# FelipeMartins96/rsoccer-isaac-cleanrl

Hardware: AMD Instinct MI355X
Metric: env-steps/s (num_envs×horizon) at 65 536 envs; PPO wall-clock to 1e8 steps (higher is better)
Workload: dtype f32; 1 GPU; vss_step FULL contract: 65536 fields/GPU, one launch per control step, random actions (BASELINE configs[1]/[2] shape); fields_per_gpu=65536, mode=full, agent_rows_per_field=1, launch=eager ctypes launches, parallelism=fields sharded over 1 GPU(s), no data-path collective

## Files before the change

### rsoccer-isaac-cleanrl_amd/csrc/vss_step.hip

```cpp
#include <hip/hip_runtime.h>
#include <type_traits>
#include <stdint.h>

#include "../../include/vss.h"

#pragma clang fp contract(off)

#if defined(__HIP_DEVICE_COMPILE__) && !defined(__gfx950__)
#error "vss_step.hip targets gfx950 (CDNA4) only: wait_loads() and v_permlane32_swap are gfx950 encodings"
#endif

namespace vss {

constexpr int kWave = 64;
constexpr int kFpw = 32;
constexpr int kRec = 59;

constexpr int NSUB = 2;
#define K_H 0.025f
#define K_HH 0.0125f
#define K_FIELD_HX 0.75f
#define K_FIELD_HY 0.65f
#define K_GOAL_HY 0.2f
#define K_GOAL_BACK_X 0.85f
// ... 312 lines not shown
      ox[k] = up ? b.x[k + 3] : b.x[k];
      oy[k] = up ? b.y[k + 3] : b.y[k];
      ovx[k] = up ? b.vx[k + 3] : b.vx[k];
      ovy[k] = up ? b.vy[k + 3] : b.vy[k];
      contact_walls(ox[k], oy[k], ovx[k], ovy[k], K_ROBOT_R);
      exch(ox[k], b.x[k], b.x[k + 3]);
      exch(oy[k], b.y[k], b.y[k + 3]);
      exch(ovx[k], b.vx[k], b.vx[k + 3]);
      exch(ovy[k], b.vy[k], b.vy[k + 3]);
    }
    contact_walls(b.bx, b.by, b.bvx, b.bvy, K_BALL_R);
  }
#pragma unroll
  for (int k = 0; k < 3; ++k) {
    exch(ow[k], b.w[k], b.w[k + 3]);
    exch(oqz[k], b.qz[k], b.qz[k + 3]);
    exch(oqw[k], b.qw[k], b.qw[k + 3]);
  }
}

__device__ __forceinline__ void wait_loads() { __builtin_amdgcn_s_waitcnt(0x0F70); }

template <class T>
__device__ __forceinline__ T& at(T* base, uint32_t byte_off) {
  using B = typename std::conditional<std::is_const<T>::value, const char, char>::type;
  return *reinterpret_cast<T*>(reinterpret_cast<B*>(base) + byte_off);
}

__device__ __forceinline__ void load_bodies(const float* __restrict__ st, int64_t n, int64_t f0, int fl, Bodies& b) {
  float v[VSS_STATE_CHANNELS];
  const float* q = st + f0 + fl;
#pragma unroll
  for (int c = 0; c < VSS_STATE_CHANNELS; ++c) {
    if (c < VSS_CH_RQX || c >= VSS_CH_RQZ)
      v[c] = *q;
    q += n;
  }
  b.bx = v[VSS_CH_BALL_X]; b.by = v[VSS_CH_BALL_Y]; b.bvx = v[VSS_CH_BALL_VX]; b.bvy = v[VSS_CH_BALL_VY];
#pragma unroll
  for (int i = 0; i < 6; ++i) {
    b.x[i] = v[VSS_CH_RX + i]; b.y[i] = v[VSS_CH_RY + i]; b.qz[i] = v[VSS_CH_RQZ + i]; b.qw[i] = v[VSS_CH_RQW + i];
    b.vx[i] = v[VSS_CH_RVX + i]; b.vy[i] = v[VSS_CH_RVY + i]; b.w[i] = v[VSS_CH_RW + i];
  }
}

__device__ __forceinline__ void store_bodies(float* __restrict__ st, int64_t n, int64_t f0, int fl, const Bodies& b) {
  float v[VSS_STATE_CHANNELS];
  v[VSS_CH_BALL_X] = b.bx; v[VSS_CH_BALL_Y] = b.by; v[VSS_CH_BALL_VX] = b.bvx; v[VSS_CH_BALL_VY] = b.bvy;
#pragma unroll
  for (int i = 0; i < 6; ++i) {
    v[VSS_CH_RX + i] = b.x[i]; v[VSS_CH_RY + i] = b.y[i]; v[VSS_CH_RQZ + i] = b.qz[i]; v[VSS_CH_RQW + i] = b.qw[i];
    v[VSS_CH_RVX + i] = b.vx[i]; v[VSS_CH_RVY + i] = b.vy[i]; v[VSS_CH_RW + i] = b.w[i];
  }
  float* q = st + f0 + fl;
#pragma unroll
  for (int c = 0; c < VSS_STATE_CHANNELS; ++c) {
    if (c < VSS_CH_RQX || c >= VSS_CH_RQZ) *q = v[c];
    q += n;
  }
}

template <int W>
__device__ __forceinline__ void coop_load(const float* __restrict__ g, int nv, float* lds, int lane) {
  const int total = nv * W;
  if constexpr (W % 4 == 0) {
    const float4* g4 = reinterpret_cast<const float4*>(g);
    for (int q = lane; q < total / 4; q += kWave) {
      float4 v = at(g4, 16u * (uint32_t)q);
      int e = q * 4, fl = e / W, k = e - fl * W;
      float* d = lds + fl * kRec + k;
      d[0] = v.x; d[1] = v.y; d[2] = v.z; d[3] = v.w;
    }
  } else {
    const float2* g2 = reinterpret_cast<const float2*>(g);
    for (int q = lane; q < total / 2; q += kWave) {
      float2 v = at(g2, 8u * (uint32_t)q);
      int e = q * 2, fl = e / W, k = e - fl * W;
      float* d = lds + fl * kRec + k;
      d[0] = v.x; d[1] = v.y;
    }
  }
}

template <int W>
__device__ __forceinline__ void coop_store(float* __restrict__ g, int nv, const float* lds, int lane) {
  const int total = nv * W;
  if constexpr (W % 4 == 0) {
    float4* g4 = reinterpret_cast<float4*>(g);
    for (int q = lane; q < total / 4; q += kWave) {
      int e = q * 4, fl = e / W, k = e - fl * W;
      const float* s = lds + fl * kRec + k;
      at(g4, 16u * (uint32_t)q) = make_float4(s[0], s[1], s[2], s[3]);
    }
  } else {
    float2* g2 = reinterpret_cast<float2*>(g);
    for (int q = lane; q < total / 2; q += kWave) {
      int e = q * 2, fl = e / W, k = e - fl * W;
      const float* s = lds + fl * kRec + k;
      at(g2, 8u * (uint32_t)q) = make_float2(s[0], s[1]);
    }
  }
}

template <int A>
__device__ __forceinline__ void write_obs_record(float* rec, const Bodies& b, const float dof[12]) {
  rec[0] = b.bx; rec[1] = b.by; rec[2] = b.bvx; rec[3] = b.bvy;
#pragma unroll
  for (int r = 0; r < 6; ++r) {
    float* o = rec + 4 + 9 * r;
    o[0] = b.x[r]; o[1] = b.y[r]; o[2] = b.vx[r]; o[3] = b.vy[r];
    o[4] = b.qw[r] * b.qw[r] - b.qz[r] * b.qz[r];
    o[5] = 2.0f * b.qw[r] * b.qz[r];
    o[6] = b.w[r]; o[7] = dof[2 * r]; o[8] = dof[2 * r + 1];
  }
  if constexpr (A == 6) {
    float* m = rec + kRec;
#pragma unroll
    for (int k = 0; k < 4; ++k) m[k] = __uint_as_float(__float_as_uint(rec[k]) ^ 0x80000000u);
#pragma unroll
    for (int r = 0; r < 6; ++r)
#pragma unroll
      for (int q = 0; q < 6; ++q)
        m[4 + 6 * r + q] = __uint_as_float(__float_as_uint(rec[4 + 9 * r + q]) ^ 0x80000000u);
  }
}

constexpr int kObsUnroll = 4;
template <int A, int A0 = 0, int REC = obs_rec<A>()>
__device__ __forceinline__ void coop_store_obs(float* __restrict__ out, int nv, const float* lds, const uint32_t* tab,
                                               int lane, bool nt = false) {
  static_assert(A0 + A <= 6 && (A0 == 0 || REC == kRecObs6), "yellow agents read the mirror slots");
  constexpr int Q = 13 * A;
  constexpr int QD = kWave / Q, QR = kWave % Q;
  constexpr uint32_t RB = 4u * REC;
  const int total = nv * Q;
  const uint32_t rb_last = (uint32_t)(nv - 1) * RB;
  int fl = lane / Q, j4 = lane - fl * Q;
  uint32_t rb = (uint32_t)fl * RB;
  const char* L = reinterpret_cast<const char*>(lds);
  float4* o4 = reinterpret_cast<float4*>(out);
  for (int q0 = lane; q0 < total; q0 += kObsUnroll * kWave) {
    float4 v[kObsUnroll];
#pragma unroll
    for (int u = 0; u < kObsUnroll; ++u) {
      const uint2 t = reinterpret_cast<const uint2*>(tab)[13 * A0 + j4];
      const uint32_t r = rb < rb_last ? rb : rb_last;
      v[u].x = *reinterpret_cast<const float*>(L + r + (t.x & 0xffffu));
      v[u].y = *reinterpret_cast<const float*>(L + r + (t.x >> 16));
      v[u].z = *reinterpret_cast<const float*>(L + r + (t.y & 0xffffu));
      v[u].w = *reinterpret_cast<const float*>(L + r + (t.y >> 16));
      j4 += QR;
      rb += QD * RB;
      if (j4 >= Q) { j4 -= Q; rb += RB; }
    }
#pragma unroll
    for (int u = 0; u < kObsUnroll; ++u)
      if (q0 + u * kWave < total) {
        if (nt) {
          typedef float f4v __attribute__((ext_vector_type(4)));
          __builtin_nontemporal_store(f4v{v[u].x, v[u].y, v[u].z, v[u].w},
                                      reinterpret_cast<f4v*>(&at(o4, 16u * (uint32_t)(q0 + u * kWave))));
        } else {
          at(o4, 16u * (uint32_t)(q0 + u * kWave)) = v[u];
        }
      }
  }
}

struct ResetDraws {
  uint32_t k0, k1, field, ctr, ext;
  const float* u;
  uint32_t rounds;
};

template <bool REPLAY>
__device__ __forceinline__ float uval(uint32_t w) { return REPLAY ? __uint_as_float(w) : u01(w); }

template <bool REPLAY>
__device__ __forceinline__ void pos_block(const ResetDraws& d, uint32_t round, uint32_t blk, uint32_t o[4]) {
  if constexpr (REPLAY) {
#pragma unroll
    for (uint32_t i = 0; i < 4; ++i) {
      const uint32_t j = 4u * blk + i;
      o[i] = j < 14u ? __float_as_uint(d.u[14u * round + j]) : 0x3f000000u;
    }
  } else {
    philox(d.k0, d.k1, d.field, d.ctr, ((kPurposePos | d.ext) << 24) | round, blk, o);
  }
}

template <bool REPLAY>
__device__ __forceinline__ void ang_block(const ResetDraws& d, uint32_t rounds_used, uint32_t blk, uint32_t o[4]) {
  if constexpr (REPLAY) {
#pragma unroll
    for (uint32_t i = 0; i < 4; ++i) o[i] = __float_as_uint(d.u[14u * rounds_used + 4u * blk + i]);
  } else {
    philox(d.k0, d.k1, d.field, d.ctr, ((kPurposeAng | d.ext) << 24), blk, o);
  }
}

template <bool REPLAY>
__device__ __forceinline__ void reset_field(Bodies& b, const ResetDraws& d) {
  const float scale_x = 1.5f - 0.14f, scale_y = 1.3f - 0.14f;
  float px[7], py[7];
  uint32_t round = 0;
  for (;; ++round) {
    uint32_t o[16];
#pragma unroll
    for (int blk = 0; blk < 4; ++blk) pos_block<REPLAY>(d, round, (uint32_t)blk, o + 4 * blk);
#pragma unroll
    for (int e = 0; e < 7; ++e) {
      px[e] = (uval<REPLAY>(o[2 * e]) - 0.5f) * scale_x;
      py[e] = (uval<REPLAY>(o[2 * e + 1]) - 0.5f) * scale_y;
    }
    bool close = false;
#pragma unroll
    for (int i = 0; i < 7; ++i)
#pragma unroll
      for (int j = i + 1; j < 7; ++j) {
        float dx = px[i] - px[j], dy = py[i] - py[j];
        close |= dx * dx + dy * dy < __uint_as_float(0x3ba0902du);
      }
    if (!close || round + 1 >= d.rounds) break;
  }
  b.bx = px[0]; b.by = py[0];
  uint32_t o[8];
  ang_block<REPLAY>(d, round + 1, 0u, o);
  ang_block<REPLAY>(d, round + 1, 1u, o + 4);
#pragma unroll
  for (int r = 0; r < 6; ++r) {
    b.x[r] = px[1 + r]; b.y[r] = py[1 + r];
    b.vx[r] = 0.0f; b.vy[r] = 0.0f; b.w[r] = 0.0f;
    float ang = K_TWO_PI * uval<REPLAY>(o[r]) + (-K_PI);
    float sh, ch;
    sincos_small(ang * 0.5f, sh, ch);
    float nrm = sqrtf(sh * sh + ch * ch);
    b.qz[r] = sh / nrm;
    b.qw[r] = ch / nrm;
  }
  b.bvx = uval<REPLAY>(o[6]) - 0.5f;
  b.bvy = uval<REPLAY>(o[7]) - 0.5f;
}

template <bool REPLAY>
__device__ __forceinline__ void reset_field_split(Bodies& b, const ResetDraws& d) {
  const float kMinDist2 = __uint_as_float(0x3ba0902du);
  const bool up = threadIdx.x >= 32;
  const uint32_t blk0 = up ? 2u : 0u;
// ... 128 lines not shown
  const float u1 = u01_open0(w1), u2 = u01(w2);
  const float rad = sqrtf(-2.0f * logf_poly(u1));
  float sz, cz;
  sincos_turn(u2, sz, cz);
  zc = K_OU_SIGMA * (rad * cz);
  zs = K_OU_SIGMA * (rad * sz);
}

template <int MODE>
__device__ __forceinline__ void ou_noise_split(float a[12], uint32_t k0, uint32_t k1, uint32_t field, uint32_t ctr) {
  const bool up = threadIdx.x >= 32;
  float z[12];
  if constexpr (MODE == VSS_MODE_SA) {
    uint32_t p[4], q[4];
    philox(k0, k1, field, ctr, kPurposeOU << 24, up ? 2u : 0u, p);
    philox(k0, k1, field, ctr, kPurposeOU << 24, up ? 2u : 1u, q);
    float c0, s0, c1, s1, c2, s2;
    box_muller(up ? p[0] : p[2], up ? p[1] : p[3], c0, s0);
    box_muller(up ? p[2] : q[0], up ? p[3] : q[1], c1, s1);
    box_muller(q[2], q[3], c2, s2);
    exch(c0, z[2], z[8]);
    exch(s0, z[3], z[9]);
    exch(c1, z[4], z[10]);
    exch(s1, z[5], z[11]);
    float unused;
    exch(c2, z[6], unused);
    exch(s2, z[7], unused);
  } else {
    uint32_t p[4];
    philox(k0, k1, field, ctr, kPurposeOU << 24, up ? 2u : 1u, p);
    float c0, s0, c1, s1;
    box_muller(up ? p[0] : p[2], up ? p[1] : p[3], c0, s0);
    box_muller(p[2], p[3], c1, s1);
    exch(c0, z[6], z[8]);
    exch(s0, z[7], z[9]);
    float unused;
    exch(c1, unused, z[10]);
    exch(s1, unused, z[11]);
  }
  constexpr int NL = MODE == VSS_MODE_SA ? 2 : 6;
#pragma unroll
  for (int k = NL; k < 12; ++k) a[k] = clampf((a[k] - K_OU_THETA * a[k]) + z[k], -1.0f, 1.0f);
}

__device__ __forceinline__ void ou_noise_blue_sa(float a[12], uint32_t k0, uint32_t k1, uint32_t field, uint32_t ctr) {
  const bool up = threadIdx.x >= 32;
  uint32_t w[4];
  philox(k0, k1, field, ctr, kPurposeOU << 24, up ? 1u : 0u, w);
  float zc, zs, z[6];
  box_muller(up ? w[0] : w[2], up ? w[1] : w[3], zc, zs);
  exch(zc, z[2], z[4]);
  exch(zs, z[3], z[5]);
#pragma unroll
  for (int k = 2; k < 6; ++k) a[k] = clampf((a[k] - K_OU_THETA * a[k]) + z[k], -1.0f, 1.0f);
}

template <bool REPLAY>
__device__ __forceinline__ void reset_if_done(bool valid, int64_t done, const ResetDraws& rd, Bodies& b,
                                              const float a[12], float dof[12]) {
#pragma unroll
  for (int k = 0; k < 12; ++k) dof[k] = a[k];
  if (valid && done) {
    reset_field_split<REPLAY>(b, rd);
#pragma unroll
    for (int k = 0; k < 12; ++k) dof[k] = dof[k] * 0.0f;
  }
}

struct BatchIn {
  int64_t progress, reset_prev;
  uint32_t ctr;
  Bodies b;
  float4 blk[3];
  float2 lrn[2];
};

struct StepArgs {
  int64_t n;
  vss_params p;
  vss_state s;
  vss_step_io io;
  vss_replay_draws rd;
  uint32_t rd_rounds;
  uint32_t nt_obs;
};

template <int MODE>
__device__ __forceinline__ void load_batch(const StepArgs& args, int64_t f0, int nv, int fl, int lane, BatchIn& in) {
  constexpr int NL = MODE == VSS_MODE_SA ? 2 : 6;
  in.progress = 0;
  in.reset_prev = 0;
  in.ctr = 0;
  in.b = {};
  if (fl < nv) {
    in.progress = at(args.s.progress_buf + f0, 8u * (uint32_t)fl);
    in.reset_prev = at(args.s.reset_buf + f0, 8u * (uint32_t)fl);
    in.ctr = at(args.s.rng_counter + f0, 4u * (uint32_t)fl);
    load_bodies(args.s.state, args.n, f0, fl, in.b);
  }
  prefetch12((MODE == VSS_MODE_FULL ? args.io.actions : args.io.ou_buf) + f0 * 12, nv, lane, in.blk);
  if constexpr (MODE != VSS_MODE_FULL) prefetch_lrn<NL>(args.io.actions + f0 * NL, nv, lane, in.lrn);
}

template <int MODE, bool REPLAY, bool VERSUS, bool MIRROR = false>
__device__ __forceinline__ void step_body(const StepArgs& args, const vss_versus_io& vs,
                                          const vss_mirror_io& yl = vss_mirror_io{}) {
  static_assert(!VERSUS || (!REPLAY && (MODE == VSS_MODE_SA || MODE == VSS_MODE_CMA || MODE == VSS_MODE_DMA)),
                "versus: wrapped modes only, no replay");
  static_assert(!MIRROR || (!REPLAY && !VERSUS && (MODE == VSS_MODE_SA || MODE == VSS_MODE_CMA || MODE == VSS_MODE_DMA)),
                "mirror: wrapped modes only, no replay, not versus");
  constexpr bool TWO = VERSUS || MIRROR;
  constexpr int A = MODE == VSS_MODE_FULL ? 6 : (MODE == VSS_MODE_DMA ? 3 : 1);
  constexpr int R = MODE == VSS_MODE_DMA ? 3 : 1;
  constexpr int NL = MODE == VSS_MODE_SA ? 2 : 6;
  constexpr int REC = TWO ? kRecObs6 : obs_rec<A>();
  static_assert(2 * kFpw == kWave, "two lanes per field");
  constexpr int kLds = 32 * kRec > kFpw * REC ? 32 * kRec : kFpw * REC;
  static_assert(kFpw * REC <= kLds, "observation records must fit the LDS block");
  __shared__ float lds[kLds + kTabWords];
  uint32_t* tab = reinterpret_cast<uint32_t*>(lds + kLds);
  stage_obs_table(tab, threadIdx.x);

  const int64_t n = args.n;
  const int lane = threadIdx.x;
  const int fl = lane & 31;
  const bool writer = lane < 32;
  const uint32_t k0 = (uint32_t)args.p.seed, k1 = (uint32_t)(args.p.seed >> 32);
  float* rec = lds + fl * kRec;
  float* orec = lds + lane * REC;

  const int64_t f0 = (int64_t)blockIdx.x * kFpw;
  const int nv = (int)(n - f0 < kFpw ? n - f0 : kFpw);
  BatchIn cur;
  load_batch<MODE>(args, f0, nv, fl, lane, cur);
  float2 opp[2];
  if constexpr (VERSUS) prefetch_lrn<6>(vs.opp_actions + f0 * 6, nv, lane, opp);
  if constexpr (MIRROR) prefetch_lrn<NL>(yl.actions + f0 * NL, nv, lane, opp);
  const int64_t f = f0 + fl;
  const bool valid = fl < nv;
  const bool owner = valid && writer;

  int64_t progress = cur.progress;
  const uint32_t ctr = cur.ctr;
  Bodies b = cur.b;

  float a[12];
  stage12(cur.blk, nv, lds, lane);
  __syncthreads();
#pragma unroll
  for (int k = 0; k < 12; ++k) a[k] = rec[k];
  __syncthreads();

  float ou[12];
  if constexpr (MODE != VSS_MODE_FULL) {
    if constexpr (VERSUS) {
      if constexpr (MODE == VSS_MODE_SA) ou_noise_blue_sa(a, k0, k1, (uint32_t)f, ctr);
    } else if constexpr (MIRROR) {
      if constexpr (MODE == VSS_MODE_SA) ou_noise_split<MODE>(a, k0, k1, (uint32_t)f, ctr);
    } else if constexpr (REPLAY) {
      if (valid) {
        const float* z = args.rd.normals + f * 12;
#pragma unroll
        for (int k = NL; k < 12; ++k) a[k] = clampf((a[k] - K_OU_THETA * a[k]) + z[k], -1.0f, 1.0f);
      }
    } else {
      ou_noise_split<MODE>(a, k0, k1, (uint32_t)f, ctr);
    }
    stage_lrn<NL>(cur.lrn, nv, lds, lane);
    if constexpr (VERSUS) stage_lrn<6>(opp, nv, lds + 6, lane);
    if constexpr (MIRROR) stage_lrn<NL>(opp, nv, lds + 6, lane);
    __syncthreads();
#pragma unroll
    for (int k = 0; k < NL; ++k) a[k] = rec[k];
    if constexpr (VERSUS) {
#pragma unroll
      for (int k = 6; k < 12; ++k) a[k] = rec[k];
    }
    if constexpr (MIRROR) {
#pragma unroll
      for (int k = 6; k < 6 + NL; ++k) a[k] = rec[k];
    }
    __syncthreads();
#pragma unroll
    for (int k = 0; k < 12; ++k) ou[k] = a[k];
  }

  const float clip = args.p.clip_actions;
#pragma unroll
  for (int k = 0; k < 12; ++k) a[k] = clampf(a[k], -clip, clip);
  if (cur.reset_prev != 0) progress = 0;

  float pbx = b.bx, pby = b.by, prx[6], pry[6];
#pragma unroll
  for (int i = 0; i < 6; ++i) { prx[i] = b.x[i]; pry[i] = b.y[i]; }

  if (valid) physics_split(b, a);

  progress += 1;
  float rew[24];
  const int64_t done = rewards_and_done(args.p, b, pbx, pby, prx, pry, a, progress, rew);

  wait_loads();

  if (lane < kFpw) write_obs_record<MIRROR ? 6 : A>(orec, b, a);
  __syncthreads();
  coop_store_obs<A, 0, REC>(args.io.terminal_obs + f0 * (52 * A), nv, lds, tab, lane, MODE != VSS_MODE_FULL);
  if constexpr (MIRROR) coop_store_obs<A, 3, REC>(yl.terminal_obs + f0 * (52 * A), nv, lds, tab, lane, true);
  __syncthreads();

  float dof[12];
  const ResetDraws rd{k0, k1, (uint32_t)f, ctr, 0u, REPLAY ? args.rd.uniforms + f * args.rd.uniform_stride : nullptr,
                      REPLAY ? args.rd_rounds : (uint32_t)kMaxRejectRounds};
  reset_if_done<REPLAY>(valid, done, rd, b, a, dof);

  if (lane < kFpw) write_obs_record<TWO ? 6 : A>(orec, b, dof);
  __syncthreads();
  coop_store_obs<A, 0, REC>(args.io.obs + f0 * (52 * A), nv, lds, tab, lane, MODE != VSS_MODE_FULL || args.nt_obs != 0);
  if constexpr (VERSUS) coop_store_obs<3, 3, REC>(vs.opp_obs + f0 * (52 * 3), nv, lds, tab, lane, true);
  if constexpr (MIRROR) coop_store_obs<A, 3, REC>(yl.obs + f0 * (52 * A), nv, lds, tab, lane, true);
  __syncthreads();

  const uint8_t time_out = (progress >= (int64_t)args.p.max_episode_length - 1) && done != 0;
  if (owner) {
    const uint32_t ufl = (uint32_t)fl;
    store_bodies(args.s.state, n, f0, fl, b);
    at(args.s.progress_buf + f0, 8u * ufl) = progress;
    at(args.s.reset_buf + f0, 8u * ufl) = done;
    at(args.s.rng_counter + f0, 4u * ufl) = ctr + 1u;
#pragma unroll
    for (int k = 0; k < R; ++k) {
      at(args.io.time_outs + f0 * R, (uint32_t)(ufl * R + k)) = time_out;
      at(args.io.progress_f + f0 * R, 4u * (ufl * R + k)) = (float)progress;
    }
    if constexpr (MODE == VSS_MODE_DMA && !MIRROR) {
#pragma unroll
      for (int k = 0; k < 3; ++k) at(args.io.dones_rep + f0 * 3, 8u * (ufl * 3 + k)) = done;
    }
    if constexpr (MIRROR) {
#pragma unroll
      for (int k = 0; k < R; ++k) {
        at(args.io.dones_rep + f0 * R, 8u * (ufl * R + k)) = done;
        at(yl.dones + f0 * R, 8u * (ufl * R + k)) = done;
        at(yl.time_outs + f0 * R, (uint32_t)(ufl * R + k)) = time_out;
        at(yl.progress_f + f0 * R, 4u * (ufl * R + k)) = (float)progress;
      }
    }
  }

  if (writer) {
#pragma unroll
    for (int k = 0; k < 12; ++k) rec[k] = dof[k];
  }
  __syncthreads();
  coop_store<12>(args.s.dof_velocity_buf + f0 * 12, nv, lds, lane);
  __syncthreads();
  if constexpr (MODE != VSS_MODE_FULL) {
    if (writer) {
#pragma unroll
      for (int k = 0; k < 12; ++k) rec[k] = done ? ou[k] * 0.0f : ou[k];
    }
    __syncthreads();
    coop_store<12>(args.io.ou_buf + f0 * 12, nv, lds, lane);
    __syncthreads();
  }

  if constexpr (MODE == VSS_MODE_FULL) {
    if (writer) {
#pragma unroll
      for (int k = 0; k < 24; ++k) rec[k] = rew[k];
    }
    __syncthreads();
    coop_store<24>(args.io.rew + f0 * 24, nv, lds, lane);
    if (owner && args.io.reward_sum) at(args.io.reward_sum + f0, 4u * (uint32_t)fl) = ((rew[0] + rew[1]) + rew[2]) + rew[3];
  } else if constexpr (MODE == VSS_MODE_SA) {
    if (owner) {
      at(reinterpret_cast<float4*>(args.io.rew) + f0, 16u * (uint32_t)fl) = make_float4(rew[0], rew[1], rew[2], rew[3]);
      at(args.io.reward_sum + f0, 4u * (uint32_t)fl) = ((rew[0] + rew[1]) + rew[2]) + rew[3];
      if constexpr (MIRROR) {
        at(reinterpret_cast<float4*>(yl.rew) + f0, 16u * (uint32_t)fl) = make_float4(rew[12], rew[13], rew[14], rew[15]);
        at(yl.reward_sum + f0, 4u * (uint32_t)fl) = ((rew[12] + rew[13]) + rew[14]) + rew[15];
      }
    }
  } else if constexpr (MODE == VSS_MODE_CMA) {
    if (owner) {
      float m[4];
#pragma unroll
      for (int c = 0; c < 4; ++c) m[c] = ((rew[c] + rew[4 + c]) + rew[8 + c]) / 3.0f;
      at(reinterpret_cast<float4*>(args.io.rew) + f0, 16u * (uint32_t)fl) = make_float4(m[0], m[1], m[2], m[3]);
      at(args.io.reward_sum + f0, 4u * (uint32_t)fl) = ((m[0] + m[1]) + m[2]) + m[3];
      if constexpr (MIRROR) {
        float y[4];
#pragma unroll
        for (int c = 0; c < 4; ++c) y[c] = ((rew[12 + c] + rew[16 + c]) + rew[20 + c]) / 3.0f;
        at(reinterpret_cast<float4*>(yl.rew) + f0, 16u * (uint32_t)fl) = make_float4(y[0], y[1], y[2], y[3]);
        at(yl.reward_sum + f0, 4u * (uint32_t)fl) = ((y[0] + y[1]) + y[2]) + y[3];
      }
    }
  } else {
    if (writer) {
#pragma unroll
      for (int k = 0; k < 12; ++k) rec[k] = rew[k];
    }
    __syncthreads();
    coop_store<12>(args.io.rew + f0 * 12, nv, lds, lane);
    if (owner) {
#pragma unroll
      for (int ag = 0; ag < 3; ++ag)
        at(args.io.reward_sum + f0 * 3, 4u * ((uint32_t)fl * 3 + ag)) =
            ((rew[4 * ag] + rew[4 * ag + 1]) + rew[4 * ag + 2]) + rew[4 * ag + 3];
    }
    if constexpr (MIRROR) {
      __syncthreads();
      if (writer) {
#pragma unroll
        for (int k = 0; k < 12; ++k) rec[k] = rew[12 + k];
      }
      __syncthreads();
      coop_store<12>(yl.rew + f0 * 12, nv, lds, lane);
      if (owner) {
#pragma unroll
        for (int ag = 0; ag < 3; ++ag)
          at(yl.reward_sum + f0 * 3, 4u * ((uint32_t)fl * 3 + ag)) =
              ((rew[12 + 4 * ag] + rew[13 + 4 * ag]) + rew[14 + 4 * ag]) + rew[15 + 4 * ag];
      }
    }
  }
}

template <int MODE, bool REPLAY = false>
__global__ __launch_bounds__(kWave) void step_kernel(StepArgs args) {
  step_body<MODE, REPLAY, false>(args, vss_versus_io{});
}

template <int MODE>
__global__ __launch_bounds__(kWave) void step_versus_kernel(StepArgs args, vss_versus_io vs) {
  step_body<MODE, false, true>(args, vs);
}

template <int MODE>
__global__ __launch_bounds__(kWave) void step_mirror_kernel(StepArgs args, vss_mirror_io yl) {
  step_body<MODE, false, false, true>(args, vss_versus_io{}, yl);
}

struct RolloutArgs {
  int64_t n;
  int32_t k_steps;
  vss_params p;
  vss_state s;
  vss_rollout_io io;
};

__global__ __launch_bounds__(kWave) void rollout_kernel(RolloutArgs args) {
  static_assert(kFpw * kRecObs6 <= kWave * kRec, "observation records must fit the LDS block");
  __shared__ float lds[kWave * kRec + kTabWords];
  uint32_t* tab = reinterpret_cast<uint32_t*>(lds + kWave * kRec);
  stage_obs_table(tab, threadIdx.x);
  const int64_t n = args.n;
  const int lane = threadIdx.x;
  const int fl = lane & (kFpw - 1);
  const int64_t f0 = (int64_t)blockIdx.x * kFpw;
  const int nv = (int)(n - f0 < kFpw ? n - f0 : kFpw);
  const int64_t f = f0 + fl;
  const bool valid = fl < nv;
  const bool owner = valid && lane < kFpw;
  const bool writer = lane < kFpw;
  const uint32_t k0 = (uint32_t)args.p.seed, k1 = (uint32_t)(args.p.seed >> 32);
  float* rec = lds + fl * kRec;
  float* orec = lds + lane * kRecObs6;

  int64_t progress = 0, reset_prev = 0;
  uint32_t ctr = 0;
  Bodies b = {};
  if (valid) {
    progress = at(args.s.progress_buf + f0, 8u * (uint32_t)fl);
    reset_prev = at(args.s.reset_buf + f0, 8u * (uint32_t)fl);
    ctr = at(args.s.rng_counter + f0, 4u * (uint32_t)fl);
    load_bodies(args.s.state, n, f0, fl, b);
  }
  float4 pre[3];
  prefetch12(args.io.actions + f0 * 12, nv, lane, pre);
  float dof[12];
  int64_t done = reset_prev;
  const float clip = args.p.clip_actions;

  for (int k = 0; k < args.k_steps; ++k) {
    const int64_t step_off = (int64_t)k * n;
    float a[12];
    stage12(pre, nv, lds, lane);
    __syncthreads();
#pragma unroll
    for (int i = 0; i < 12; ++i) a[i] = clampf(rec[i], -clip, clip);
    __syncthreads();
    if (k + 1 < args.k_steps) prefetch12(args.io.actions + (step_off + n + f0) * 12, nv, lane, pre);

    if (reset_prev != 0) progress = 0;
    float pbx = b.bx, pby = b.by, prx[6], pry[6];
#pragma unroll
    for (int i = 0; i < 6; ++i) { prx[i] = b.x[i]; pry[i] = b.y[i]; }
    if (valid) {
      physics_split(b, a);
    }
    progress += 1;
    float rew[24];
    done = rewards_and_done(args.p, b, pbx, pby, prx, pry, a, progress, rew);

    wait_loads();
    if (lane < kFpw) write_obs_record<6>(orec, b, a);
    __syncthreads();
    coop_store_obs<6>(args.io.terminal_obs + (step_off + f0) * 312, nv, lds, tab, lane, true);
    __syncthreads();
    const ResetDraws rd{k0, k1, (uint32_t)f, ctr + (uint32_t)k, 0u, nullptr, (uint32_t)kMaxRejectRounds};
    reset_if_done<false>(valid, done, rd, b, a, dof);
    if (lane < kFpw) write_obs_record<6>(orec, b, dof);
    __syncthreads();
    coop_store_obs<6>(args.io.obs + (step_off + f0) * 312, nv, lds, tab, lane, true);
    __syncthreads();
    if (writer) {
#pragma unroll
      for (int i = 0; i < 24; ++i) rec[i] = rew[i];
    }
    __syncthreads();
    coop_store<24>(args.io.rew + (step_off + f0) * 24, nv, lds, lane);
    __syncthreads();
    if (owner) {
      args.io.dones[step_off + f] = done;
      args.io.time_outs[step_off + f] = (progress >= (int64_t)args.p.max_episode_length - 1) && done != 0;
      args.io.progress_f[step_off + f] = (float)progress;
    }
    reset_prev = done;
  }

  if (owner) {
    store_bodies(args.s.state, n, f0, fl, b);
    args.s.progress_buf[f] = progress;
    args.s.reset_buf[f] = done;
    args.s.rng_counter[f] = ctr + (uint32_t)args.k_steps;
  }
  if (writer) {
#pragma unroll
    for (int i = 0; i < 12; ++i) rec[i] = dof[i];
  }
  __syncthreads();
  coop_store<12>(args.s.dof_velocity_buf + f0 * 12, nv, lds, lane);
}

template <bool REPLAY>
__global__ __launch_bounds__(kWave) void reset_kernel(int64_t n, vss_params p, vss_state s, vss_replay_draws rdr,
                                                     uint32_t rounds) {
  const int64_t f = (int64_t)blockIdx.x * kWave + threadIdx.x;
  if (f >= n || s.reset_buf[f] == 0) return;
  Bodies b;
  const int64_t f0 = (int64_t)blockIdx.x * kWave;
  load_bodies(s.state, n, f0, (int)threadIdx.x, b);
  const uint32_t ctr = s.rng_counter[f];
  const ResetDraws rd{(uint32_t)p.seed, (uint32_t)(p.seed >> 32), (uint32_t)f, ctr, kExternal,
                      REPLAY ? rdr.uniforms + f * rdr.uniform_stride : nullptr, REPLAY ? rounds : (uint32_t)kMaxRejectRounds};
  reset_field<REPLAY>(b, rd);
  store_bodies(s.state, n, f0, (int)threadIdx.x, b);
  s.rng_counter[f] = ctr + 1u;
#pragma unroll
  for (int k = 0; k < 12; ++k) s.dof_velocity_buf[f * 12 + k] = s.dof_velocity_buf[f * 12 + k] * 0.0f;
}

template <int A>
__global__ __launch_bounds__(kWave) void observe_kernel(int64_t n, vss_state s, float* obs) {
  __shared__ float lds[kWave * obs_rec<A>() + kTabWords];
  uint32_t* tab = reinterpret_cast<uint32_t*>(lds + kWave * obs_rec<A>());
  stage_obs_table(tab, threadIdx.x);
  const int lane = threadIdx.x;
  const int64_t f0 = (int64_t)blockIdx.x * kWave;
  const int nv = (int)(n - f0 < kWave ? n - f0 : kWave);

  float* rec = lds + lane * kRec;
  float* orec = lds + lane * obs_rec<A>();
  coop_load<12>(s.dof_velocity_buf + f0 * 12, nv, lds, lane);
  __syncthreads();
  float dof[12];
#pragma unroll
  for (int k = 0; k < 12; ++k) dof[k] = rec[k];
  __syncthreads();
  Bodies b = {};
  if (lane < nv) {
    load_bodies(s.state, n, f0, lane, b);
    write_obs_record<A>(orec, b, dof);
  }
  wait_loads();
  __syncthreads();
  coop_store_obs<A>(obs + f0 * (52 * A), nv, lds, tab, lane);
}

__global__ __launch_bounds__(256) void episode_stats_kernel(int64_t rows, const float4* __restrict__ rews,
                                                            const int64_t* __restrict__ dones, float4* ep_ret,
                                                            int32_t* ep_len, float4* __restrict__ ret_out,
                                                            int32_t* __restrict__ len_out, float* __restrict__ sum_out) {
  const int64_t i = (int64_t)blockIdx.x * blockDim.x + threadIdx.x;
  if (i >= rows) return;
  const float4 r = rews[i];
  float4 e = ep_ret[i];
// ... 2 lines not shown
  ret_out[i] = e;
  len_out[i] = l;
  sum_out[i] = ((e.x + e.y) + e.z) + e.w;
  const int64_t keep = 1 - dones[i];
  const float kf = (float)keep;
  ep_ret[i] = make_float4(e.x * kf, e.y * kf, e.z * kf, e.w * kf);
  ep_len[i] = (int32_t)(l * keep);
}

__global__ __launch_bounds__(256) void match_tally_kernel(int64_t n_fields, int rows_per_field, int64_t group_fields,
                                                          const float4* __restrict__ rew,
                                                          const int64_t* __restrict__ dones,
                                                          const float* __restrict__ progress_f,
                                                          unsigned long long* tally) {
  const int64_t f = (int64_t)blockIdx.x * blockDim.x + threadIdx.x;
  const int lane = threadIdx.x & 63;
  bool done = false;
  int q = 0;
  float goal = 0.0f;
  long long steps = 0;
  if (f < n_fields) {
    const int64_t r = f * rows_per_field;
    done = dones[r] != 0;
    if (done) {
      q = (int)(f / group_fields);
      goal = rew[r].x;
      steps = (long long)progress_f[r];
    }
  }
  unsigned long long todo = __ballot(done);
  while (todo) {
    const int leader = __ffsll(todo) - 1;
    const int qq = __shfl(q, leader);
    const bool mine = done && q == qq;
    const unsigned long long m = __ballot(mine);
    const unsigned long long won = __ballot(mine && goal > 0.0f);
    const unsigned long long lost = __ballot(mine && goal < 0.0f);
    long long s = mine ? steps : 0;
#pragma unroll
    for (int d = 32; d >= 1; d >>= 1) s += __shfl_xor(s, d);
    if (lane == leader) {
      unsigned long long* t = tally + 4 * qq;
      atomicAdd(t + 0, (unsigned long long)__popcll(m));
      if (won) atomicAdd(t + 1, (unsigned long long)__popcll(won));
      if (lost) atomicAdd(t + 2, (unsigned long long)__popcll(lost));
      atomicAdd(t + 3, (unsigned long long)s);
    }
    todo &= ~m;
  }
}

}

static bool bad(const void* ptr, uintptr_t align) { return !ptr || (reinterpret_cast<uintptr_t>(ptr) & (align - 1)); }
static bool misaligned(const void* ptr, uintptr_t align) { return ptr && (reinterpret_cast<uintptr_t>(ptr) & (align - 1)); }

static int check_state(int64_t n, const vss_state* st) {
  if (n < 0 || n > (int64_t(1) << 26) || !st) return VSS_E_ARG;
  if (bad(st->state, 4) || bad(st->progress_buf, 8) || bad(st->reset_buf, 8) || bad(st->dof_velocity_buf, 16) ||
      bad(st->rng_counter, 4))
    return VSS_E_ARG;
  return VSS_OK;
}

static int launch_status() { return hipGetLastError() == hipSuccess ? VSS_OK : VSS_E_LAUNCH; }

static int replay_rounds(const vss_replay_draws* d) {
  if (!d || bad(d->uniforms, 4) || d->uniform_stride < 22 || d->uniform_stride > (int64_t(1) << 20)) return -1;
  const int64_t r = (d->uniform_stride - 8) / 14;
  return r > vss::kMaxRejectRounds ? -1 : (int)r;
}

static int check_step_io(int32_t mode, const vss_step_io* io) {
  const bool wrapped = mode != VSS_MODE_FULL;
  if (bad(io->actions, wrapped ? 8 : 16) || bad(io->obs, 16) || bad(io->terminal_obs, 16) || bad(io->rew, 16) ||
      bad(io->time_outs, 1) || bad(io->progress_f, 4) || misaligned(io->reward_sum, 4) ||
      misaligned(io->ou_buf, 16) || misaligned(io->dones_rep, 8))
    return VSS_E_ARG;
  if (wrapped && (!io->ou_buf || !io->reward_sum)) return VSS_E_ARG;
  if (mode == VSS_MODE_DMA && !io->dones_rep) return VSS_E_ARG;
  return VSS_OK;
}

template <bool REPLAY, bool VERSUS, bool MIRROR = false>
static int launch_step(void* stream, int64_t n, int32_t mode, const vss_params* p, const vss_state* st,
                       const vss_step_io* io, const vss_replay_draws* rd, int rounds, const vss_versus_io* vs,
                       const vss_mirror_io* yl = nullptr) {
  if (n == 0) return VSS_OK;
  const uint32_t nt_obs = mode == VSS_MODE_FULL && n > (int64_t)(256ll << 20) / 3101 ? 1u : 0u;
  vss::StepArgs args{n, *p, *st, *io, REPLAY ? *rd : vss_replay_draws{}, (uint32_t)rounds, nt_obs};
  const dim3 grid((unsigned)((n + vss::kFpw - 1) / vss::kFpw)), block(vss::kWave);
  hipStream_t s = (hipStream_t)stream;
  auto launch = [&](auto m) {
    constexpr int MODE = decltype(m)::value;
    if constexpr (VERSUS) hipLaunchKernelGGL((vss::step_versus_kernel<MODE>), grid, block, 0, s, args, *vs);
    else if constexpr (MIRROR) hipLaunchKernelGGL((vss::step_mirror_kernel<MODE>), grid, block, 0, s, args, *yl);
    else hipLaunchKernelGGL((vss::step_kernel<MODE, REPLAY>), grid, block, 0, s, args);
  };
  switch (mode) {
    case VSS_MODE_FULL:
      if constexpr (!VERSUS && !MIRROR) launch(std::integral_constant<int, VSS_MODE_FULL>{});
      break;
    case VSS_MODE_SA: launch(std::integral_constant<int, VSS_MODE_SA>{}); break;
    case VSS_MODE_CMA: launch(std::integral_constant<int, VSS_MODE_CMA>{}); break;
    default: launch(std::integral_constant<int, VSS_MODE_DMA>{}); break;
  }
  return launch_status();
}

template <bool REPLAY>
static int step_impl(void* stream, int64_t n, int32_t mode, const vss_params* p, const vss_state* st,
                     const vss_step_io* io, const vss_replay_draws* rd) {
  if (int rc = check_state(n, st)) return rc;
  if (!p || !io || mode < VSS_MODE_FULL || mode > VSS_MODE_DMA) return VSS_E_ARG;
  if (int rc = check_step_io(mode, io)) return rc;
  int rounds = 0;
  if (REPLAY) {
    rounds = replay_rounds(rd);
    if (rounds < 1 || (mode != VSS_MODE_FULL && bad(rd->normals, 4))) return VSS_E_ARG;
  }
  return launch_step<REPLAY, false>(stream, n, mode, p, st, io, rd, rounds, nullptr);
}

extern "C" {

int vss_abi_version(void) { return VSS_ABI_VERSION; }

const char* vss_error_string(int code) {
  switch (code) {
    case VSS_OK: return "ok";
    case VSS_E_ARG: return "invalid argument (null or misaligned buffer, bad size or bad mode)";
    case VSS_E_LAUNCH: return "kernel launch failed";
    default: return "unknown error";
  }
}

int vss_step(void* stream, int64_t n, int32_t mode, const vss_params* p, const vss_state* st,
             const vss_step_io* io) {
  return step_impl<false>(stream, n, mode, p, st, io, nullptr);
}

int vss_step_replay(void* stream, int64_t n, int32_t mode, const vss_params* p, const vss_state* st,
                    const vss_step_io* io, const vss_replay_draws* draws) {
  return step_impl<true>(stream, n, mode, p, st, io, draws);
}

int vss_step_versus(void* stream, int64_t n, int32_t mode, const vss_params* p, const vss_state* st,
                    const vss_step_io* io, const vss_versus_io* vs) {
  if (int rc = check_state(n, st)) return rc;
  if (!p || !io || !vs || mode < VSS_MODE_SA || mode > VSS_MODE_DMA) return VSS_E_ARG;
  if (int rc = check_step_io(mode, io)) return rc;
  if (bad(vs->opp_actions, 8) || bad(vs->opp_obs, 16)) return VSS_E_ARG;
  return launch_step<false, true>(stream, n, mode, p, st, io, nullptr, 0, vs);
}

int vss_step_mirror(void* stream, int64_t n, int32_t mode, const vss_params* p, const vss_state* st,
                    const vss_step_io* io, const vss_mirror_io* yl) {
  if (int rc = check_state(n, st)) return rc;
  if (!p || !io || !yl || mode < VSS_MODE_SA || mode > VSS_MODE_DMA) return VSS_E_ARG;
  if (int rc = check_step_io(mode, io)) return rc;
  if (!io->dones_rep) return VSS_E_ARG;
  if (bad(yl->actions, 8) || bad(yl->obs, 16) || bad(yl->terminal_obs, 16) || bad(yl->rew, 16) ||
      bad(yl->reward_sum, 4) || bad(yl->dones, 8) || bad(yl->time_outs, 1) || bad(yl->progress_f, 4))
    return VSS_E_ARG;
  return launch_step<false, false, true>(stream, n, mode, p, st, io, nullptr, 0, nullptr, yl);
}

int vss_rollout(void* stream, int64_t n, int32_t k_steps, const vss_params* p, const vss_state* st,
                const vss_rollout_io* io) {
  if (int rc = check_state(n, st)) return rc;
  if (!p || !io || k_steps < 1 || k_steps > (1 << 20)) return VSS_E_ARG;
  if (bad(io->actions, 16) || bad(io->obs, 16) || bad(io->terminal_obs, 16) || bad(io->rew, 16) ||
      bad(io->dones, 8) || bad(io->time_outs, 1) || bad(io->progress_f, 4))
// ... 72 lines not shown
```

Baseline: 1.695 billion env-steps/s.

## Route step-kernel stores through buffer resources with per-group cache policies

Replaces global float4 stores in the observation, reward and dof-velocity writers with raw buffer stores. These carry a runtime-selected cache policy (plain, nontemporal, write-through, or write-through plus nontemporal) chosen per output group from the problem size and mode. It also adds an optional wave-cooperative, LDS-transposed store of body state. The aim is to keep outputs that the next step or the PPO consumer rereads resident in the last-level cache when the footprint fits, and to stream them otherwise. The cost is a runtime policy switch around each store loop and more code paths, and the right policy depends on the actual cache size. The bounds check in coop_store_obs is dropped in favour of buffer-resource range clamping.

```diff
diff --git a/rsoccer-isaac-cleanrl_amd/csrc/vss_step.hip b/rsoccer-isaac-cleanrl_amd/csrc/vss_step.hip
--- a/rsoccer-isaac-cleanrl_amd/csrc/vss_step.hip
+++ b/rsoccer-isaac-cleanrl_amd/csrc/vss_step.hip
@@ -418,16 +418,82 @@
   }
 }
 
+enum : uint32_t { kStPlain = 0, kStNt = 1, kStWt = 2, kStWtNt = 3 };
+enum : uint32_t { kGrpTerminal = 0, kGrpObs = 2, kGrpYellow = 4, kGrpState = 6, kGrpAos = 8 };
+constexpr uint32_t policy_word(uint32_t terminal, uint32_t obs, uint32_t yellow, uint32_t state, uint32_t aos) {
+  return terminal << kGrpTerminal | obs << kGrpObs | yellow << kGrpYellow | state << kGrpState | aos << kGrpAos;
+}
+__device__ __forceinline__ uint32_t policy_of(uint32_t word, uint32_t grp) { return (word >> grp) & 3u; }
+
+using BufRsrc = __amdgpu_buffer_rsrc_t;
+__device__ __forceinline__ BufRsrc wave_rsrc(void* base, uint32_t bytes) {
+  return __builtin_amdgcn_make_buffer_rsrc(base, 0, (int)bytes, 0x00020000);
+}
+
+template <uint32_t POL>
+__device__ __forceinline__ void store16(BufRsrc r, uint32_t off, float4 v) {
+  typedef uint32_t u4v __attribute__((ext_vector_type(4)));
+  constexpr int aux = POL == kStNt ? 2 : POL == kStWt ? 16 : POL == kStWtNt ? 18 : 0;
+  const u4v d = {__float_as_uint(v.x), __float_as_uint(v.y), __float_as_uint(v.z), __float_as_uint(v.w)};
+  __builtin_amdgcn_raw_buffer_store_b128(d, r, (int)off, 0, aux);
+}
+
+template <class F>
+__device__ __forceinline__ void with_policy(uint32_t pol, F f) {
+  switch (pol) {
+    case kStNt: f(std::integral_constant<uint32_t, kStNt>{}); break;
+    case kStWt: f(std::integral_constant<uint32_t, kStWt>{}); break;
+    case kStWtNt: f(std::integral_constant<uint32_t, kStWtNt>{}); break;
+    default: f(std::integral_constant<uint32_t, kStPlain>{}); break;
+  }
+}
+
+__device__ __forceinline__ void store_bodies_wave(float* __restrict__ st, int64_t n, int64_t f0, const Bodies& b,
+                                                  float* lds, int lane, bool writer, uint32_t pol) {
+  constexpr int kLive = VSS_STATE_CHANNELS - (VSS_CH_RQZ - VSS_CH_RQX);
+  static_assert(kLive <= kRec && kFpw == 32, "one record per field, eight 16-B pieces per channel");
+  if (writer) {
+    float* r = lds + lane * kRec;
+    r[VSS_CH_BALL_X] = b.bx; r[VSS_CH_BALL_Y] = b.by; r[VSS_CH_BALL_VX] = b.bvx; r[VSS_CH_BALL_VY] = b.bvy;
+    constexpr int D = VSS_CH_RQZ - VSS_CH_RQX;
+#pragma unroll
+    for (int i = 0; i < 6; ++i) {
+      r[VSS_CH_RX + i] = b.x[i]; r[VSS_CH_RY + i] = b.y[i];
+      r[VSS_CH_RQZ - D + i] = b.qz[i]; r[VSS_CH_RQW - D + i] = b.qw[i];
+      r[VSS_CH_RVX - D + i] = b.vx[i]; r[VSS_CH_RVY - D + i] = b.vy[i]; r[VSS_CH_RW - D + i] = b.w[i];
+    }
+  }
+  __syncthreads();
+  const uint32_t un = (uint32_t)n;
+  const BufRsrc rs = wave_rsrc(st + f0, 4u * ((uint32_t)(VSS_STATE_CHANNELS - 1) * un + (uint32_t)kFpw));
+  with_policy(pol, [&](auto P) {
+#pragma unroll
+    for (int i = 0; i < (kLive * 8 + kWave - 1) / kWave; ++i) {
+      const int s = lane + i * kWave, ci = s >> 3, part = s & 7;
+      if (ci < kLive) {
+        const uint32_t c = (uint32_t)(ci < VSS_CH_RQX ? ci : ci + (VSS_CH_RQZ - VSS_CH_RQX));
+        const float* src = lds + (part * 4) * kRec + ci;
+        store16<decltype(P)::value>(rs, 4u * (c * un) + 16u * (uint32_t)part,
+                                    make_float4(src[0], src[kRec], src[2 * kRec], src[3 * kRec]));
+      }
+    }
+  });
+  __syncthreads();
+}
+
 template <int W>
-__device__ __forceinline__ void coop_store(float* __restrict__ g, int nv, const float* lds, int lane) {
+__device__ __forceinline__ void coop_store(float* __restrict__ g, int nv, const float* lds, int lane,
+                                           uint32_t pol = kStPlain) {
   const int total = nv * W;
   if constexpr (W % 4 == 0) {
-    float4* g4 = reinterpret_cast<float4*>(g);
-    for (int q = lane; q < total / 4; q += kWave) {
-      int e = q * 4, fl = e / W, k = e - fl * W;
-      const float* s = lds + fl * kRec + k;
-      at(g4, 16u * (uint32_t)q) = make_float4(s[0], s[1], s[2], s[3]);
-    }
+    const BufRsrc rs = wave_rsrc(g, 4u * (uint32_t)total);
+    with_policy(pol, [&](auto P) {
+      for (int q = lane; q < total / 4; q += kWave) {
+        int e = q * 4, fl = e / W, k = e - fl * W;
+        const float* s = lds + fl * kRec + k;
+        store16<decltype(P)::value>(rs, 16u * (uint32_t)q, make_float4(s[0], s[1], s[2], s[3]));
+      }
+    });
   } else {
     float2* g2 = reinterpret_cast<float2*>(g);
     for (int q = lane; q < total / 2; q += kWave) {
@@ -464,7 +530,7 @@
 constexpr int kObsUnroll = 4;
 template <int A, int A0 = 0, int REC = obs_rec<A>()>
 __device__ __forceinline__ void coop_store_obs(float* __restrict__ out, int nv, const float* lds, const uint32_t* tab,
-                                               int lane, bool nt = false) {
+                                               int lane, uint32_t pol = kStPlain) {
   static_assert(A0 + A <= 6 && (A0 == 0 || REC == kRecObs6), "yellow agents read the mirror slots");
   constexpr int Q = 13 * A;
   constexpr int QD = kWave / Q, QR = kWave % Q;
@@ -474,8 +540,9 @@
   int fl = lane / Q, j4 = lane - fl * Q;
   uint32_t rb = (uint32_t)fl * RB;
   const char* L = reinterpret_cast<const char*>(lds);
-  float4* o4 = reinterpret_cast<float4*>(out);
-  for (int q0 = lane; q0 < total; q0 += kObsUnroll * kWave) {
+  const BufRsrc rs = wave_rsrc(out, 16u * (uint32_t)total);
+  for (int base = 0; base < total; base += kObsUnroll * kWave) {
+    const int q0 = base + lane;
     float4 v[kObsUnroll];
 #pragma unroll
     for (int u = 0; u < kObsUnroll; ++u) {
@@ -489,17 +556,10 @@
       rb += QD * RB;
       if (j4 >= Q) { j4 -= Q; rb += RB; }
     }
-#pragma unroll
-    for (int u = 0; u < kObsUnroll; ++u)
-      if (q0 + u * kWave < total) {
-        if (nt) {
-          typedef float f4v __attribute__((ext_vector_type(4)));
-          __builtin_nontemporal_store(f4v{v[u].x, v[u].y, v[u].z, v[u].w},
-                                      reinterpret_cast<f4v*>(&at(o4, 16u * (uint32_t)(q0 + u * kWave))));
-        } else {
-          at(o4, 16u * (uint32_t)(q0 + u * kWave)) = v[u];
-        }
-      }
+    with_policy(pol, [&](auto P) {
+#pragma unroll
+      for (int u = 0; u < kObsUnroll; ++u) store16<decltype(P)::value>(rs, 16u * (uint32_t)(q0 + u * kWave), v[u]);
+    });
   }
 }
 
@@ -794,7 +854,7 @@
   vss_step_io io;
   vss_replay_draws rd;
   uint32_t rd_rounds;
-  uint32_t nt_obs;
+  uint32_t store_policy;
 };
 
 template <int MODE>
@@ -834,6 +894,7 @@
   stage_obs_table(tab, threadIdx.x);
 
   const int64_t n = args.n;
+  const uint32_t pol = args.store_policy;
   const int lane = threadIdx.x;
   const int fl = lane & 31;
   const bool writer = lane < 32;
@@ -916,8 +977,8 @@
 
   if (lane < kFpw) write_obs_record<MIRROR ? 6 : A>(orec, b, a);
   __syncthreads();
-  coop_store_obs<A, 0, REC>(args.io.terminal_obs + f0 * (52 * A), nv, lds, tab, lane, MODE != VSS_MODE_FULL);
-  if constexpr (MIRROR) coop_store_obs<A, 3, REC>(yl.terminal_obs + f0 * (52 * A), nv, lds, tab, lane, true);
+  coop_store_obs<A, 0, REC>(args.io.terminal_obs + f0 * (52 * A), nv, lds, tab, lane, policy_of(pol, kGrpTerminal));
+  if constexpr (MIRROR) coop_store_obs<A, 3, REC>(yl.terminal_obs + f0 * (52 * A), nv, lds, tab, lane, policy_of(pol, kGrpYellow));
   __syncthreads();
 
   float dof[12];
@@ -927,15 +988,17 @@
 
   if (lane < kFpw) write_obs_record<TWO ? 6 : A>(orec, b, dof);
   __syncthreads();
-  coop_store_obs<A, 0, REC>(args.io.obs + f0 * (52 * A), nv, lds, tab, lane, MODE != VSS_MODE_FULL || args.nt_obs != 0);
-  if constexpr (VERSUS) coop_store_obs<3, 3, REC>(vs.opp_obs + f0 * (52 * 3), nv, lds, tab, lane, true);
-  if constexpr (MIRROR) coop_store_obs<A, 3, REC>(yl.obs + f0 * (52 * A), nv, lds, tab, lane, true);
+  coop_store_obs<A, 0, REC>(args.io.obs + f0 * (52 * A), nv, lds, tab, lane, policy_of(pol, kGrpObs));
+  if constexpr (VERSUS) coop_store_obs<3, 3, REC>(vs.opp_obs + f0 * (52 * 3), nv, lds, tab, lane, policy_of(pol, kGrpYellow));
+  if constexpr (MIRROR) coop_store_obs<A, 3, REC>(yl.obs + f0 * (52 * A), nv, lds, tab, lane, policy_of(pol, kGrpYellow));
   __syncthreads();
 
   const uint8_t time_out = (progress >= (int64_t)args.p.max_episode_length - 1) && done != 0;
+  const bool state_wave = policy_of(pol, kGrpState) != kStPlain && nv == kFpw;
+  if (state_wave) store_bodies_wave(args.s.state, n, f0, b, lds, lane, writer, policy_of(pol, kGrpState));
   if (owner) {
     const uint32_t ufl = (uint32_t)fl;
-    store_bodies(args.s.state, n, f0, fl, b);
+    if (!state_wave) store_bodies(args.s.state, n, f0, fl, b);
     at(args.s.progress_buf + f0, 8u * ufl) = progress;
     at(args.s.reset_buf + f0, 8u * ufl) = done;
     at(args.s.rng_counter + f0, 4u * ufl) = ctr + 1u;
@@ -959,12 +1022,13 @@
     }
   }
 
+  const uint32_t aos = policy_of(pol, kGrpAos);
   if (writer) {
 #pragma unroll
     for (int k = 0; k < 12; ++k) rec[k] = dof[k];
   }
   __syncthreads();
-  coop_store<12>(args.s.dof_velocity_buf + f0 * 12, nv, lds, lane);
+  coop_store<12>(args.s.dof_velocity_buf + f0 * 12, nv, lds, lane, aos);
   __syncthreads();
   if constexpr (MODE != VSS_MODE_FULL) {
     if (writer) {
@@ -972,7 +1036,7 @@
       for (int k = 0; k < 12; ++k) rec[k] = done ? ou[k] * 0.0f : ou[k];
     }
     __syncthreads();
-    coop_store<12>(args.io.ou_buf + f0 * 12, nv, lds, lane);
+    coop_store<12>(args.io.ou_buf + f0 * 12, nv, lds, lane, aos);
     __syncthreads();
   }
 
@@ -982,7 +1046,7 @@
       for (int k = 0; k < 24; ++k) rec[k] = rew[k];
     }
     __syncthreads();
-    coop_store<24>(args.io.rew + f0 * 24, nv, lds, lane);
+    coop_store<24>(args.io.rew + f0 * 24, nv, lds, lane, aos);
     if (owner && args.io.reward_sum) at(args.io.reward_sum + f0, 4u * (uint32_t)fl) = ((rew[0] + rew[1]) + rew[2]) + rew[3];
   } else if constexpr (MODE == VSS_MODE_SA) {
     if (owner) {
@@ -1014,7 +1078,7 @@
       for (int k = 0; k < 12; ++k) rec[k] = rew[k];
     }
     __syncthreads();
-    coop_store<12>(args.io.rew + f0 * 12, nv, lds, lane);
+    coop_store<12>(args.io.rew + f0 * 12, nv, lds, lane, aos);
     if (owner) {
 #pragma unroll
       for (int ag = 0; ag < 3; ++ag)
@@ -1028,7 +1092,7 @@
         for (int k = 0; k < 12; ++k) rec[k] = rew[12 + k];
       }
       __syncthreads();
-      coop_store<12>(yl.rew + f0 * 12, nv, lds, lane);
+      coop_store<12>(yl.rew + f0 * 12, nv, lds, lane, aos);
       if (owner) {
 #pragma unroll
         for (int ag = 0; ag < 3; ++ag)
@@ -1119,13 +1183,13 @@
     wait_loads();
     if (lane < kFpw) write_obs_record<6>(orec, b, a);
     __syncthreads();
-    coop_store_obs<6>(args.io.terminal_obs + (step_off + f0) * 312, nv, lds, tab, lane, true);
+    coop_store_obs<6>(args.io.terminal_obs + (step_off + f0) * 312, nv, lds, tab, lane, kStNt);
     __syncthreads();
     const ResetDraws rd{k0, k1, (uint32_t)f, ctr + (uint32_t)k, 0u, nullptr, (uint32_t)kMaxRejectRounds};
     reset_if_done<false>(valid, done, rd, b, a, dof);
     if (lane < kFpw) write_obs_record<6>(orec, b, dof);
     __syncthreads();
-    coop_store_obs<6>(args.io.obs + (step_off + f0) * 312, nv, lds, tab, lane, true);
+    coop_store_obs<6>(args.io.obs + (step_off + f0) * 312, nv, lds, tab, lane, kStNt);
     __syncthreads();
     if (writer) {
 #pragma unroll
@@ -1294,13 +1358,43 @@
   return VSS_OK;
 }
 
+#define VSS_STORE_adopted 0
+#define VSS_STORE_present 1
+#define VSS_STORE_obs_wt 2
+#define VSS_STORE_all_wt 3
+#define VSS_STORE_tail_wt 4
+#define VSS_STORE_all_wtnt 5
+#define VSS_STORE_wt_aos 6
+#ifndef VSS_STEP_STORE
+#define VSS_STEP_STORE VSS_STORE_adopted
+#endif
+static uint32_t store_policy(int32_t mode, int64_t n, bool two_sided) {
+  using namespace vss;
+  const bool full = mode == VSS_MODE_FULL;
+  const bool past_cache = full && n > (int64_t)(256ll << 20) / 3101;
+  const uint32_t term = full ? kStPlain : kStNt, obs = full && !past_cache ? kStPlain : kStNt;
+  static const int64_t kBytesPerField[4] = {3101, 1001, 1017, 1923};
+  const bool fits = n <= (int64_t)(256ll << 20) / kBytesPerField[mode];
+  const bool wt = fits && (mode != VSS_MODE_DMA || two_sided);
+  uint32_t w;
+  switch (VSS_STEP_STORE == VSS_STORE_adopted ? (wt ? VSS_STORE_wt_aos : VSS_STORE_present) : VSS_STEP_STORE) {
+    case VSS_STORE_obs_wt: w = policy_word(kStWt, kStWt, kStWt, kStPlain, kStPlain); break;
+    case VSS_STORE_all_wt: w = policy_word(kStWt, kStWt, kStWt, kStWt, kStWt); break;
+    case VSS_STORE_tail_wt: w = policy_word(term, kStWt, kStNt, kStWt, kStWt); break;
+    case VSS_STORE_all_wtnt: w = policy_word(kStWtNt, kStWtNt, kStWtNt, kStWt, kStWt); break;
+    case VSS_STORE_wt_aos: w = policy_word(kStWt, kStWt, kStWt, kStPlain, kStWt); break;
+    default: w = policy_word(term, obs, kStNt, kStPlain, kStPlain); break;
+  }
+  if (n > (int64_t(1) << 23)) w &= ~(3u << kGrpState);
+  return w;
+}
+
 template <bool REPLAY, bool VERSUS, bool MIRROR = false>
 static int launch_step(void* stream, int64_t n, int32_t mode, const vss_params* p, const vss_state* st,
                        const vss_step_io* io, const vss_replay_draws* rd, int rounds, const vss_versus_io* vs,
                        const vss_mirror_io* yl = nullptr) {
   if (n == 0) return VSS_OK;
-  const uint32_t nt_obs = mode == VSS_MODE_FULL && n > (int64_t)(256ll << 20) / 3101 ? 1u : 0u;
-  vss::StepArgs args{n, *p, *st, *io, REPLAY ? *rd : vss_replay_draws{}, (uint32_t)rounds, nt_obs};
+  vss::StepArgs args{n, *p, *st, *io, REPLAY ? *rd : vss_replay_draws{}, (uint32_t)rounds, store_policy(mode, n, VERSUS || MIRROR)};
   const dim3 grid((unsigned)((n + vss::kFpw - 1) / vss::kFpw)), block(vss::kWave);
   hipStream_t s = (hipStream_t)stream;
   auto launch = [&](auto m) {
```

New measurement: 1.836 billion env-steps/s, median of 6. 1.08x the previous value.
